# ErrorTzy/unpaper-gpu

Measured on AMD Instinct MI355X. Metric: pages/sec + Mpixel/s, 1000-page GRAY8 A4@300dpi batch, 1/2/4/8 GPU, higher is better.
Workload: dtype u8; 1 GPU; 1000 synthetic GRAY8 A4@300dpi pages (2480x3508) per GPU, default pipeline, inputs and outputs resident in HBM; pages_per_gpu=1000, sheets_per_batch=64, streams=16, hw_queues=24, parallelism=one runner thread per device, pages sharded, no collective

## Files before the change

unpaper-gpu_amd/csrc/kernels_noise.hip:

```cpp
#include "filters_common.h"

namespace uph {

constexpr int kNT = 64;
constexpr int kHalo = 14;
constexpr int kRW = kNT + 2 * kHalo;
constexpr int kNTG = 100;
template <int FMT>
constexpr int noise_tile_w() { return FMT == F_GRAY8 ? kNTG : kNT; }
constexpr int kZone = 32;
constexpr int kEligible = kZone + 8;

bool noise_geometry(int32_t W, int32_t H, uint64_t intensity, uint8_t white, NoiseGeom* g) {
  g->W = W;
  g->H = H;
  g->intensity = intensity > 64 ? 64 : (int32_t)intensity;
  g->white = white;
  g->all_seq = intensity > 4 ? 1 : 0;
  int64_t cap = g->all_seq ? (int64_t)W * H + 64 : ((int64_t)W * H) / 4 + 1024;
  if (cap > (1 << 27)) cap = 1 << 27;
  g->capacity = (int32_t)cap;
  return true;
}

static size_t noise_list_bytes(const NoiseGeom& g) {
  size_t b = 256 + (size_t)g.capacity * 4 * 2;
  return (b + 255) & ~(size_t)255;
}

static size_t pow2_at_least(size_t n) {
  size_t p = 1;
  while (p < n) p <<= 1;
  return p;
}

static int32_t noise_bit_words(const NoiseGeom& g) { return noise_bit_words(g.W); }

constexpr int kCapPerThread = 16;
static int group_threads(int32_t W, int32_t H) { return (int64_t)W * H > (16 << 20) ? 1024 : 256; }
size_t noise_scratch_bytes(const NoiseGeom& g) {
  size_t sort = 4 * pow2_at_least((size_t)g.capacity);
  const size_t cap3 = 12 * (size_t)kCapPerThread * (size_t)group_threads(g.W, g.H);
  if (sort < cap3) sort = cap3;
  const size_t bits = 4 * (size_t)noise_bit_words(g) * (size_t)g.H;
  return noise_list_bytes(g) + (sort > bits ? sort : bits);
}

struct NoisePtrs {
  uint32_t* nclear;
  uint32_t* nseq;
  uint32_t* clear;
  uint32_t* seq;
};
__device__ __forceinline__ NoisePtrs noise_ptrs(const NoiseGeom& g, uint8_t* base) {
  NoisePtrs p;
  p.nclear = (uint32_t*)base;
  p.nseq = p.nclear + 1;
  p.clear = (uint32_t*)(base + 256);
  p.seq = p.clear + g.capacity;
  return p;
}

__device__ __forceinline__ uint32_t row9(const uint32_t* w, int c) {
  const int word = c >> 5, off = c & 31;
  uint64_t v = ((uint64_t)w[word + 1] << 32) | w[word];
  return (uint32_t)(v >> off) & 0x1FFu;
}

__device__ __forceinline__ int flood9(const uint32_t (*drow)[4], int cx, int cy, uint32_t* comp) {
  uint32_t D[9], cur[9];
#pragma unroll
  for (int r = 0; r < 9; r++) {
    D[r] = row9(drow[cy - 4 + r], cx - 4);
    cur[r] = 0;
  }
  cur[4] = 1u << 4;
  for (int it = 0; it < 4; it++) {
    uint32_t nx[9];
    bool same = true;
    int n = 0;
#pragma unroll
    for (int r = 0; r < 9; r++) {
      uint32_t u = cur[r] | (r > 0 ? cur[r - 1] : 0) | (r < 8 ? cur[r + 1] : 0);
      u = (u | (u << 1) | (u >> 1)) & D[r] & 0x1FFu;
      nx[r] = u;
      same &= (u == cur[r]);
      n += __popc(u);
    }
#pragma unroll
    for (int r = 0; r < 9; r++) cur[r] = nx[r];
    if (n > 4) {
#pragma unroll
      for (int r = 0; r < 9; r++) comp[r] = cur[r];
      return n;
    }
    if (same) break;
  }
  int n = 0;
#pragma unroll
  for (int r = 0; r < 9; r++) {
    comp[r] = cur[r];
    n += __popc(cur[r]);
  }
  return n;
}

__device__ __forceinline__ uint32_t row_bits(const uint32_t* w, int c, int n) {
  const int word = c >> 5, off = c & 31;
  const uint64_t v = ((uint64_t)(word < 3 ? w[word + 1] : 0u) << 32) | w[word];
  return (uint32_t)(v >> off) & (n >= 32 ? 0xFFFFFFFFu : ((1u << n) - 1u));
}

__device__ __forceinline__ void wave_append(bool want, int32_t gx, int32_t gy, uint32_t* counter,
                                            uint32_t* list, int32_t capacity) {
  const unsigned long long M = __ballot(want);
  if (!M) return;
  const int lane = threadIdx.x & 63;
  uint32_t base = 0;
  const int leader = __ffsll((long long)M) - 1;
  if (lane == leader) base = atomicAdd(counter, (uint32_t)__popcll(M));
  base = __shfl(base, leader, 64);
  if (want) {
    const uint32_t k = base + (uint32_t)__popcll(M & ((1ull << lane) - 1ull));
    if (k < (uint32_t)capacity) list[k] = ((uint32_t)gy << 16) | (uint32_t)gx;
  }
}

__global__ void __launch_bounds__(256) k_noise_bits(PlaneRef img, NoiseGeom g, uint32_t* bits,
                                                    int64_t bstride, int32_t nwr, float rnwr) {
  const int s = blockIdx.y;
  const int32_t t = blockIdx.x * 256 + threadIdx.x;
  int32_t y = (int32_t)((float)t * rnwr);
  if (y * nwr > t) y--;
  else if ((y + 1) * nwr <= t) y++;
  if (y >= g.H) return;
  const int32_t wi = t - y * nwr, x0 = 32 * wi;
  const uint4* p = reinterpret_cast<const uint4*>(plane_ptr(img, s) + (int64_t)y * img.P.pitch + x0);
  const uint4 a = p[0], b = p[1];
  uint32_t m = dark_bits32({a.x, a.y, a.z, a.w, b.x, b.y, b.z, b.w}, g.white);
  if (x0 + 32 > g.W) m &= (1u << (g.W - x0)) - 1u;
  bits[s * bstride + t] = m;
}

struct SmallVerdict {
  bool seq, clear;
};
constexpr uint32_t kNotSmall = 0xFFFFFFFFu;
__device__ __forceinline__ uint32_t pack_comp(const uint32_t (&comp)[9]) {
  uint32_t rec = kNotSmall;
  int nc = 0;
#pragma unroll
  for (int r = 0; r < 9; r++) {
    uint32_t mm = comp[r];
    while (mm) {
      const int b = __ffs(mm) - 1;
      mm &= mm - 1;
      if (nc < 4) rec = (rec & ~(0xFFu << (8 * nc))) | ((uint32_t)(b | (r << 4)) << (8 * nc));
      nc++;
    }
  }
  return nc <= 4 ? rec : kNotSmall;
}
__device__ __forceinline__ SmallVerdict small_verdict_pixels(const uint32_t (*drow)[4],
                                                             const uint32_t (*trow)[4],
                                                             const uint32_t (*srow)[4], int rx,
                                                             int ry, int32_t gx, int32_t gy,
                                                             bool trig, int N, int nc,
                                                             const int (&cxs)[4],
                                                             const int (&cys)[4]) {
  SmallVerdict v{false, false};
  int bx0 = 4, bx1 = -4, by0 = 4, by1 = -4;
#pragma unroll
  for (int k = 0; k < 4; k++)
    if (k < nc) {
      bx0 = imin(bx0, cxs[k]);
      bx1 = imax(bx1, cxs[k]);
      by0 = imin(by0, cys[k]);
      by1 = imax(by1, cys[k]);
    }
  bool eligible = nc <= 4 && gx + bx0 >= kEligible && gy + by0 >= kEligible;
  if (eligible) {
    const int X0 = rx + bx0 - 7, n = bx1 - bx0 + 15;
    const int r0 = ry + by0 - 7, r1 = ry + by1 + 7;
    int cnt = 0;
#pragma unroll
    for (int j = 0; j < 18; j++)
      if (r0 + j <= r1) cnt += __popc(row_bits(srow[r0 + j], X0, n));
    eligible = cnt == nc;
  }
  if (!eligible) {
    v.seq = trig;
    return v;
  }
  for (int k = 0; k < nc && k < 4 && !v.clear; k++) {
    const int cx = rx + (k == 0 ? cxs[0] : k == 1 ? cxs[1] : k == 2 ? cxs[2] : cxs[3]);
    const int cy = ry + (k == 0 ? cys[0] : k == 1 ? cys[1] : k == 2 ? cys[2] : cys[3]);
    if (!((trow[cy][cx >> 5] >> (cx & 31)) & 1)) continue;
    uint32_t D[9];
#pragma unroll
    for (int r = 0; r < 9; r++) D[r] = row_bits(drow[cy - 4 + r], cx - 4, 9);
    int count = 1;
    bool go = true;
#pragma unroll
    for (int L = 1; L <= 4; L++) {
      if (!go || L > N) break;
      const uint32_t span = ((1u << (2 * L + 1)) - 1u) << (4 - L);
      const uint32_t ends = (1u << (4 - L)) | (1u << (4 + L));
      int lc = __popc(D[4 - L] & span) + __popc(D[4 + L] & span);
#pragma unroll
      for (int r = 4 - L + 1; r <= 4 + L - 1; r++) lc += __popc(D[r] & ends);
      count += lc;
      go = lc != 0;
    }
    v.clear = count <= N;
  }
  return v;
}
__device__ __forceinline__ SmallVerdict small_verdict_rec(const uint32_t (*drow)[4],
                                                          const uint32_t (*trow)[4],
                                                          const uint32_t (*srow)[4], int rx, int ry,
                                                          int32_t gx, int32_t gy, bool trig, int N,
                                                          uint32_t rec) {
  int cxs[4], cys[4], nc = 0;
#pragma unroll
  for (int k = 0; k < 4; k++) {
    const uint32_t b = (rec >> (8 * k)) & 0xFFu;
    cxs[k] = (int)(b & 15u) - 4;
    cys[k] = (int)(b >> 4) - 4;
    nc += b != 0xFFu;
  }
  return small_verdict_pixels(drow, trow, srow, rx, ry, gx, gy, trig, N, nc, cxs, cys);
}
__device__ __forceinline__ SmallVerdict small_verdict(const uint32_t (*drow)[4],
                                                      const uint32_t (*trow)[4],
                                                      const uint32_t (*srow)[4], int rx, int ry,
                                                      int32_t gx, int32_t gy, bool trig, int N) {
  uint32_t comp[9];
  flood9(drow, rx, ry, comp);
  const uint32_t rec = pack_comp(comp);
  if (rec == kNotSmall) return SmallVerdict{trig, false};
  return small_verdict_rec(drow, trow, srow, rx, ry, gx, gy, trig, N, rec);
}

constexpr int kListCap = 1024;

#ifndef UPH_CLASSIFY_OCC
#define UPH_CLASSIFY_OCC 8
#endif
template <int FMT>
__global__ void __launch_bounds__(256, UPH_CLASSIFY_OCC) k_noise_classify(PlaneRef img, NoiseGeom g, uint8_t* scratch,
                                                        int64_t sstride, SheetCtl* ctl,
                                                        const uint32_t* bits, int64_t bstride) {
  int bxi, byi, s;
  xcd_block(&bxi, &byi, &s);
  constexpr int NTX = noise_tile_w<FMT>();
  constexpr int RWX = NTX + 2 * kHalo;
  static_assert(RWX > 64 && RWX <= 128, "region rows are two 64-bit halves");
  const int32_t tx0 = bxi * NTX, ty0 = byi * kNT;
  const int32_t ox = tx0 - kHalo, oy = ty0 - kHalo;
  const uint8_t* base = plane_ptr(img, s);
  NoisePtrs NP = noise_ptrs(g, scratch + s * sstride);
  const int lane = threadIdx.x & 63, w = threadIdx.x >> 6;
  constexpr bool kGray = FMT == F_GRAY8;
  constexpr bool kSplit = FMT == F_RGB24;
  constexpr uint64_t kIn0 = ~0ull << kHalo;
  constexpr uint64_t kIn1 = (1ull << (kHalo + NTX - 64)) - 1ull;
  __shared__ uint32_t drow[kRW][4];
  __shared__ uint32_t trow_s[kSplit ? kRW : 1][4];
  __shared__ uint32_t srow[kRW][4];
  __shared__ uint64_t l3[kRW][2], cand[kRW][2];
  __shared__ uint16_t wl[kListCap];
  __shared__ uint32_t crec[kListCap];
  __shared__ int32_t any_dark, nwl;
  uint32_t (*trow)[4] = kSplit ? trow_s : drow;
  constexpr int B = FMT == F_GRAY8 ? 1 : FMT == F_Y400A ? 2 : 3;
  const int64_t pitch = img.P.pitch;
  if (threadIdx.x == 0) {
    any_dark = 0;
    nwl = 0;
  }
  for (int i = threadIdx.x; i < kRW * 4; i += 256) (&srow[0][0])[i] = 0;
  if constexpr (kGray) {
    bool dark_here = false;
    if (threadIdx.x < kRW) {
      const int ry = threadIdx.x;
      const int32_t gy = oy + ry;
      const int32_t nwr = (g.W + 31) >> 5;
      const int32_t wb = ox >> 5;
      const int sh = ox & 31;
      uint32_t q[5] = {0u, 0u, 0u, 0u, 0u};
      if (gy >= 0 && gy < g.H) {
        const uint32_t* row = bits + s * bstride + (int64_t)gy * nwr;
#pragma unroll
        for (int j = 0; j < 5; j++)
          if (wb + j >= 0 && wb + j < nwr) q[j] = row[wb + j];
      }
      uint32_t d[4];
#pragma unroll
      for (int j = 0; j < 4; j++) d[j] = __builtin_amdgcn_alignbit(q[j + 1], q[j], sh);
      if (RWX < 128) {
        if (RWX <= 96) {
          d[2] &= RWX > 64 ? (1u << (RWX - 64)) - 1u : 0u;
          d[3] = 0u;
        } else {
          d[3] &= (1u << (RWX - 96)) - 1u;
        }
      }
#pragma unroll
      for (int j = 0; j < 4; j++) drow[ry][j] = d[j];
      const uint64_t lo64 = ((uint64_t)d[1] << 32) | d[0], hi64 = ((uint64_t)d[3] << 32) | d[2];
      dark_here = ry >= kHalo && ry < kHalo + kNT && ((lo64 & kIn0) | (hi64 & kIn1));
    }
    __syncthreads();
    if (dark_here) any_dark = 1;
  } else {
    constexpr int NV = (RWX * B + 30) / 16;
    constexpr int NLOAD = (kRW * NV + 255) / 256;
    __shared__ uint4 stage[kRW][NV];
    const int64_t sb = (int64_t)ox * B;
    const int64_t a0 = sb >= 0 ? (sb & ~(int64_t)15) : -((-sb + 15) & ~(int64_t)15);
    uint4 v[NLOAD];
#pragma unroll
    for (int k = 0; k < NLOAD; k++) {
      const int i = threadIdx.x + k * 256;
      const int ry = i / NV, vi = i % NV;
      const int32_t gy = oy + ry;
      const int64_t off = a0 + 16 * vi;
      v[k] = make_uint4(0, 0, 0, 0);
      if (i < kRW * NV && gy >= 0 && gy < g.H && off >= 0 && off < pitch)
        v[k] = *reinterpret_cast<const uint4*>(base + (int64_t)gy * pitch + off);
    }
#pragma unroll
    for (int k = 0; k < NLOAD; k++) {
      const int i = threadIdx.x + k * 256;
      if (i < kRW * NV) stage[i / NV][i % NV] = v[k];
    }
    __syncthreads();
    const int lead = (int)(sb - a0);
    bool colok[2];
    int rxc[2];
#pragma unroll
    for (int h = 0; h < 2; h++) {
      const int rx = h * 64 + lane;
      colok[h] = (rx < RWX) & (ox + rx >= 0) & (ox + rx < g.W);
      rxc[h] = rx < RWX ? rx : 0;
    }
    bool tile_dark = false;
    for (int ry = w; ry < kRW; ry += 4) {
      const int32_t gy = oy + ry;
      const bool rowok = (gy >= 0) & (gy < g.H);
      const uint8_t* srow_b = reinterpret_cast<const uint8_t*>(stage[ry]) + lead;
      unsigned long long md[2], mt[2];
#pragma unroll
      for (int h = 0; h < 2; h++) {
        const bool in = colok[h] & rowok;
        if constexpr (kSplit) {
          const Px p = load_px_row<FMT>(srow_b, rxc[h]);
          md[h] = __ballot(in & (light_of(p) < g.white));
          mt[h] = __ballot(in & (dark_of(p) < g.white));
        } else {
          const uint32_t v = srow_b[rxc[h] * B];
          md[h] = mt[h] = __ballot(in & (v < (uint32_t)g.white));
        }
      }
      if (lane < 4) {
        const unsigned long long q = md[lane >> 1];
        drow[ry][lane] = (uint32_t)(lane & 1 ? q >> 32 : q);
        if (kSplit) {
          const unsigned long long t = mt[lane >> 1];
          trow[ry][lane] = (uint32_t)(lane & 1 ? t >> 32 : t);
        }
      }
      if (ry >= kHalo && ry < kHalo + kNT && ((md[0] & kIn0) | (md[1] & kIn1))) tile_dark = true;
    }
    if (lane == 0 && tile_dark) any_dark = 1;
  }
  __syncthreads();
  if (!any_dark) return;
  if (UPH_DIAG_BITS(g.diag, 3) == 1) return;
  const int hr = threadIdx.x >> 1, hh = threadIdx.x & 1;
  auto dark64 = [&](int r, int h) -> uint64_t {
    return ((uint64_t)drow[r][2 * h + 1] << 32) | drow[r][2 * h];
  };
  if (threadIdx.x < 2 * kRW) {
    uint64_t c0 = 0, c1 = 0, c2 = 0, c3 = 0;
#pragma unroll
    for (int d = -1; d <= 1; d++) {
      const int r = hr + d;
      uint64_t v0 = 0, v1 = 0;
      if (r >= 0 && r < kRW) {
        v0 = dark64(r, 0);
        v1 = dark64(r, 1);
      }
      const uint64_t v = hh ? v1 : v0;
      const uint64_t Lw = hh ? (v1 << 1) | (v0 >> 63) : v0 << 1;
      const uint64_t Rw = hh ? v1 >> 1 : (v0 >> 1) | (v1 << 63);
      const uint64_t s0 = v ^ Lw ^ Rw;
      const uint64_t s1 = (v & Lw) | (v & Rw) | (Lw & Rw);
      const uint64_t k0 = c0 & s0;
      c0 ^= s0;
      const uint64_t t1 = c1 ^ s1;
      const uint64_t k1 = (c1 & s1) | (t1 & k0);
      c1 = t1 ^ k0;
      const uint64_t k2 = c2 & k1;
      c2 ^= k1;
      c3 |= k2;
    }
    l3[hr][hh] = dark64(hr, hh) & (c3 | (c2 & (c1 | c0)));
  }
  __syncthreads();
  if (threadIdx.x < 2 * kRW) {
    uint64_t c = 0;
    if (hr >= 4 && hr < kRW - 4) {
      uint64_t dil = 0;
#pragma unroll
      for (int d = -1; d <= 1; d++) {
        const uint64_t a0 = l3[hr + d][0], a1 = l3[hr + d][1];
        dil |= hh ? a1 | (a1 << 1) | (a0 >> 63) | (a1 >> 1) : a0 | (a0 << 1) | (a0 >> 1) | (a1 << 63);
      }
      c = dark64(hr, hh) & ~dil & (hh ? (1ull << (RWX - 4 - 64)) - 1ull : ~0xFull);
    }
    cand[hr][hh] = c;
    if (c) {
      int k = atomicAdd(&nwl, __popcll(c));
      while (c) {
        const int b = __ffsll((long long)c) - 1;
        c &= c - 1;
        if (k < kListCap) wl[k] = (uint16_t)((hr << 8) | (hh * 64 + b));
        k++;
      }
    }
  }
  __syncthreads();
  if (UPH_DIAG_BITS(g.diag, 3) == 2) return;
  const int ncand = nwl;
  if (ncand <= kListCap) {
    for (int i = threadIdx.x; i < ncand; i += 256) {
      const int e = wl[i], ry = e >> 8, rx = e & 0xFF;
      uint32_t comp[9];
      const bool small = flood9(drow, rx, ry, comp) <= 4;
      crec[i] = small ? pack_comp(comp) : kNotSmall;
      if (small) atomicOr(&srow[ry][rx >> 5], 1u << (rx & 31));
    }
  } else {
    for (int ry = w; ry < kRW; ry += 4) {
      unsigned long long m[2] = {0, 0};
#pragma unroll
      for (int h = 0; h < 2; h++) {
        const uint64_t c = cand[ry][h];
        if (!c) continue;
        bool small = false;
        if ((c >> lane) & 1) {
          uint32_t comp[9];
          small = flood9(drow, h * 64 + lane, ry, comp) <= 4;
        }
        m[h] = __ballot(small);
      }
      if (lane < 4) {
        const unsigned long long q = m[lane >> 1];
        srow[ry][lane] = (uint32_t)(lane & 1 ? q >> 32 : q);
      }
    }
  }
  __syncthreads();
  if (UPH_DIAG_BITS(g.diag, 3) == 3) return;
  const int N = g.intensity;
  const bool zone_tile = g.all_seq || tx0 < kZone || ty0 < kZone;
  if (zone_tile) {
    for (int t = w; t < kNT; t += 4) {
#pragma unroll 1
      for (int h = 0; h < (NTX + 63) / 64; h++) {
        const int ry = kHalo + t, cx = h * 64 + lane, rx = kHalo + (cx < NTX ? cx : 0);
        const int32_t gy = oy + ry, gx = ox + rx;
        const bool trig = (trow[ry][rx >> 5] >> (rx & 31)) & 1;
        const bool zone = g.all_seq || gx < kZone || gy < kZone;
        const bool dark = (drow[ry][rx >> 5] >> (rx & 31)) & 1;
        const bool noop = !g.all_seq && gx >= 8 && gy >= 7 && ((l3[ry][rx >> 6] >> (rx & 63)) & 1);
        wave_append(cx < NTX && dark & zone & trig & !noop, gx, gy, NP.nseq, NP.seq, g.capacity);
      }
    }
  }
  if (ncand <= kListCap) {
    for (int b0 = 0; b0 < ncand; b0 += 256) {
      const int i = b0 + threadIdx.x;
      SmallVerdict v{false, false};
      int32_t gx = 0, gy = 0;
      if (i < ncand) {
        const uint32_t rec = crec[i];
        const int e = wl[i], ry = e >> 8, rx = e & 0xFF;
        gx = ox + rx;
        gy = oy + ry;
        const bool inside = ry >= kHalo && ry < kHalo + kNT && rx >= kHalo && rx < kHalo + NTX;
        if (rec != kNotSmall && inside && !g.all_seq && gx >= kZone && gy >= kZone) {
          const bool trig = (trow[ry][rx >> 5] >> (rx & 31)) & 1;
          v = small_verdict_rec(drow, trow, srow, rx, ry, gx, gy, trig, N, rec);
        }
      }
      wave_append(v.seq, gx, gy, NP.nseq, NP.seq, g.capacity);
      wave_append(v.clear, gx, gy, NP.nclear, NP.clear, g.capacity);
    }
    return;
  }
  if (threadIdx.x == 0) nwl = 0;
  __syncthreads();
  constexpr int kChunks = (NTX + 31) / 32;
  static_assert(kChunks * kNT <= 256, "one thread per chunk");
  if (threadIdx.x < kChunks * kNT) {
    const int ry = kHalo + (threadIdx.x / kChunks), h = threadIdx.x % kChunks;
    uint32_t m = row_bits(srow[ry], kHalo + 32 * h, imin(32, NTX - 32 * h));
    if (m && !g.all_seq && oy + ry >= kZone) {
      const int32_t gx0 = ox + kHalo + 32 * h;
      if (gx0 < kZone) m &= kZone - gx0 >= 32 ? 0u : ~((1u << (kZone - gx0)) - 1u);
      if (m) {
        int k = atomicAdd(&nwl, __popc(m));
        while (m) {
          const int b = __ffs(m) - 1;
          m &= m - 1;
          if (k < kListCap) wl[k] = (uint16_t)((ry << 8) | (kHalo + 32 * h + b));
          k++;
        }
      }
    }
  }
  __syncthreads();
  const int nsmall = nwl;
  if (nsmall <= kListCap) {
    for (int b0 = 0; b0 < nsmall; b0 += 256) {
      const int i = b0 + threadIdx.x;
      SmallVerdict v{false, false};
      int32_t gx = 0, gy = 0;
      if (i < nsmall) {
        const int e = wl[i], ry = e >> 8, rx = e & 0xFF;
        gx = ox + rx;
        gy = oy + ry;
        const bool trig = (trow[ry][rx >> 5] >> (rx & 31)) & 1;
        v = small_verdict(drow, trow, srow, rx, ry, gx, gy, trig, N);
      }
      wave_append(v.seq, gx, gy, NP.nseq, NP.seq, g.capacity);
      wave_append(v.clear, gx, gy, NP.nclear, NP.clear, g.capacity);
    }
  } else {
    for (int t = w; t < kNT; t += 4) {
      const int ry = kHalo + t;
      uint32_t any = 0;
#pragma unroll
      for (int h = 0; h < kChunks; h++) any |= row_bits(srow[ry], kHalo + 32 * h, imin(32, NTX - 32 * h));
      if (!any) continue;
#pragma unroll 1
      for (int h = 0; h < (NTX + 63) / 64; h++) {
        const int cx = h * 64 + lane, rx = kHalo + (cx < NTX ? cx : 0);
        const int32_t gy = oy + ry, gx = ox + rx;
        const bool zone = g.all_seq || gx < kZone || gy < kZone;
        const bool small = cx < NTX && !zone && ((srow[ry][rx >> 5] >> (rx & 31)) & 1);
        SmallVerdict v{false, false};
        if (small) {
          const bool trig = (trow[ry][rx >> 5] >> (rx & 31)) & 1;
          v = small_verdict(drow, trow, srow, rx, ry, gx, gy, trig, N);
        }
        wave_append(v.seq, gx, gy, NP.nseq, NP.seq, g.capacity);
        wave_append(v.clear, gx, gy, NP.nclear, NP.clear, g.capacity);
      }
    }
  }
}

template <int FMT>
__device__ __forceinline__ uint32_t* sheet_bb(const NoiseGeom& g, int s) {
  return FMT == F_GRAY8 && g.bbits ? g.bbits + s * g.bb_stride : nullptr;
}
__device__ __forceinline__ void bb_clear(uint32_t* bb, int32_t W, int32_t x, int32_t y) {
  if (bb) atomicAnd(bb + (int64_t)y * ((W + 31) >> 5) + (x >> 5), ~(1u << (x & 31)));
}

template <int FMT>
__global__ void __launch_bounds__(256) k_noise_apply(PlaneRef img, NoiseGeom g, uint8_t* scratch,
                                                     int64_t sstride, SheetCtl* ctl) {
  const int s = blockIdx.y;
  NoisePtrs NP = noise_ptrs(g, scratch + s * sstride);
  const uint32_t n = *NP.nclear;
  if (n > (uint32_t)g.capacity) {
    if (blockIdx.x == 0 && threadIdx.x == 0 && ctl) atomicOr(&ctl[s].status, STATUS_NOISE_OVERFLOW);
    return;
  }
  uint8_t* base = plane_ptr(img, s);
  uint32_t* bb = sheet_bb<FMT>(g, s);
  for (uint32_t i = blockIdx.x * 256 + threadIdx.x; i < n; i += gridDim.x * 256) {
    const uint32_t k = NP.clear[i];
    white_px<FMT>(base + (int64_t)(k >> 16) * img.P.pitch, (int32_t)(k & 0xFFFF));
    bb_clear(bb, g.W, (int32_t)(k & 0xFFFF), (int32_t)(k >> 16));
  }
}

__device__ void block_sort(uint32_t* a, int n_pow2) {
  for (int k = 2; k <= n_pow2; k <<= 1) {
    int j = k >> 1;
    for (; j >= 64; j >>= 1) {
      for (int i = threadIdx.x; i < n_pow2; i += blockDim.x) {
        const int l = i ^ j;
        if (l > i) {
          const uint32_t x = a[i], y = a[l];
          const bool up = (i & k) == 0;
          if ((x > y) == up) {
            a[i] = y;
            a[l] = x;
          }
        }
      }
      __threadfence_block();
      __syncthreads();
    }
    for (int i = threadIdx.x; i < n_pow2; i += blockDim.x) {
      uint32_t x = a[i];
      const bool up = (i & k) == 0;
      for (int jj = j; jj > 0; jj >>= 1) {
        const uint32_t y = (uint32_t)__shfl_xor((int)x, jj, 64);
        const bool lower = (i & jj) == 0;
        x = lower == up ? (x < y ? x : y) : (x < y ? y : x);
      }
      a[i] = x;
    }
    __threadfence_block();
    __syncthreads();
  }
}

__device__ __forceinline__ bool ring_pos(int L, int k, int* dx, int* dy) {
  const int row = 2 * L + 1, col = 2 * L - 1;
  if (k < row) {
    *dx = k - L;
    *dy = -L;
  } else if (k < 2 * row) {
    *dx = k - row - L;
    *dy = L;
  } else if (k < 2 * row + col) {
    *dx = -L;
    *dy = k - 2 * row - (L - 1);
  } else if (k < 2 * row + 2 * col) {
    *dx = L;
    *dy = k - 2 * row - col - (L - 1);
  } else {
    return false;
  }
  return true;
}

__device__ __forceinline__ bool ring_member(int L, int dx, int dy, int32_t x, int32_t y) {
  return iabs(dy) == L ? x >= L : y >= L - 1;
}

struct Mask81 {
  uint64_t lo;
  uint32_t hi;
};
__device__ __forceinline__ Mask81 ring_part(int L, bool rows) {
  Mask81 m{0, 0};
#pragma unroll
  for (int p = 0; p < 81; p++) {
    const int dx = p % 9 - 4, dy = p / 9 - 4;
    const int adx = iabs(dx), ady = iabs(dy);
    const bool on = rows ? (ady == L && adx <= L) : (adx == L && ady < L);
    if (on) {
      if (p < 64) m.lo |= 1ull << p;
      else m.hi |= 1u << (p - 64);
    }
  }
  return m;
}

template <int FMT>
__device__ __forceinline__ void replay_trigger4(int32_t x, int32_t y, int N, const NoiseGeom& g,
                                                uint8_t* base, int64_t pitch,
                                                const Mask81 (&rowp)[5], const Mask81 (&colp)[5],
                                                uint32_t* bb) {
  uint64_t dlo = 0;
  uint32_t dhi = 0;
  bool ctr = false;
  if constexpr (FMT == F_GRAY8) {
    const int32_t c0 = x - 4;
    const int32_t d0 = c0 >= 0 ? (c0 & ~3) : -(((-c0) + 3) & ~3);
    const int32_t dmax = (int32_t)pitch - 4;
    uint32_t w[9][3];
#pragma unroll
    for (int r = 0; r < 9; r++) {
      const uint8_t* row = base + (int64_t)imin(imax(y + r - 4, 0), g.H - 1) * pitch;
#pragma unroll
      for (int j = 0; j < 3; j++)
        w[r][j] = *reinterpret_cast<const uint32_t*>(row + imin(imax(d0 + 4 * j, 0), dmax));
    }
    const int o = c0 - d0;
#pragma unroll
    for (int p = 0; p < 81; p++) {
      const int r = p / 9, c = p % 9;
      const int32_t qx = c0 + c, qy = y + r - 4;
      const bool in = (qx >= 0) & (qy >= 0) & (qx < g.W) & (qy < g.H);
      const int b = o + c;
      const uint32_t wd = b < 4 ? w[r][0] : b < 8 ? w[r][1] : w[r][2];
      const uint32_t v = (wd >> (8 * (b & 3))) & 0xFFu;
      const bool dk = in & (v < g.white);
      if (p < 64) dlo |= (uint64_t)dk << p;
      else dhi |= (uint32_t)dk << (p - 64);
      if (p == 40) ctr = v < g.white;
    }
  } else if constexpr (FMT == F_RGB24) {
    const int32_t b0 = 3 * (x - 4);
    const int32_t d0 = b0 >= 0 ? (b0 & ~3) : -(((-b0) + 3) & ~3);
    const int32_t dmax = (int32_t)pitch - 4;
    const int o = b0 - d0;
#pragma unroll
    for (int r = 0; r < 9; r++) {
      const uint8_t* row = base + (int64_t)imin(imax(y + r - 4, 0), g.H - 1) * pitch;
      uint32_t w[8], a[7];
#pragma unroll
      for (int j = 0; j < 8; j++)
        w[j] = *reinterpret_cast<const uint32_t*>(row + imin(imax(d0 + 4 * j, 0), dmax));
#pragma unroll
// ... 322 lines not shown
    const int kb = nl <= kLongList ? (int)longs[q++] : k++;
    const int lo = (int)bc[kb], len = (int)bc[kb + 1] - lo;
    if (len <= kGroupBucketMax) continue;
    int p2 = 1;
    while (p2 < len) p2 <<= 1;
    __threadfence_block();
    __syncthreads();
    if (!BIG || p2 <= kCompCap) {
      for (int i = tid; i < p2; i += kGroupThreads) cur[i] = i < len ? keys[lo + i] : 0xFFFFFFFFu;
      __threadfence_block();
      __syncthreads();
      block_sort(cur, p2);
      for (int i = tid; i < len; i += kGroupThreads) keys[lo + i] = cur[i];
    } else {
      uint32_t* stage = NP.clear;
      for (int i = tid; i < p2; i += kGroupThreads) stage[i] = i < len ? keys[lo + i] : 0xFFFFFFFFu;
      __threadfence_block();
      __syncthreads();
      block_sort(stage, p2);
      for (int i = tid; i < len; i += kGroupThreads) keys[lo + i] = stage[i];
    }
  }
  __threadfence_block();
  __syncthreads();
  uint32_t* par = big ? NP.seq : cur;
  for (int i = tid; i < (int)n; i += kGroupThreads) par[i] = (uint32_t)i;
  __threadfence_block();
  __syncthreads();
  for (int i = tid; i < (int)n; i += kGroupThreads) {
    const uint32_t key = keys[i];
    const int32_t x = (int32_t)(key & 0xFFFF), y = (int32_t)(key >> 16);
    for (int j = (int)bc[imax(y - R, 0) >> b]; j < i; j++) {
      const uint32_t kj = keys[j];
      const int32_t xj = (int32_t)(kj & 0xFFFF), yj = (int32_t)(kj >> 16);
      if (yj >= y - R && xj >= x - R && xj <= x + R) {
        if (big) uf_union<true>(par, (uint32_t)i, (uint32_t)j);
        else uf_union(par, (uint32_t)i, (uint32_t)j);
      }
    }
  }
  __threadfence_block();
  __syncthreads();
  if (!big) {
    for (int i = tid; i < (int)n; i += kGroupThreads) {
      gk[i] = keys[i];
      gk[kCompCap + i] = uf_find(par, (uint32_t)i);
    }
    __syncthreads();
    for (int i = tid; i < (int)n; i += kGroupThreads) keys[i] = 0u;
    __syncthreads();
    for (int i = tid; i < (int)n; i += kGroupThreads) atomicMax(&keys[gk[kCompCap + i]], (uint32_t)i);
    __syncthreads();
    for (int i = tid; i < (int)n; i += kGroupThreads) gk[2 * kCompCap + i] = keys[i];
    if (tid == 0) *flag = kNoiseLds;
    return;
  }
  uint32_t* last = NP.clear;
  for (int i = tid; i < (int)n; i += kGroupThreads) last[i] = 0u;
  for (int i = tid; i < (int)n; i += kGroupThreads) par[i] = uf_find<true>(par, (uint32_t)i);
  __threadfence_block();
  __syncthreads();
  for (int i = tid; i < (int)n; i += kGroupThreads) atomicMax(&last[par[i]], (uint32_t)i);
  __threadfence();
  __syncthreads();
  if (tid == 0) *flag = kNoiseBig;
}

template <int FMT, int T>
__global__ void __launch_bounds__(T) k_noise_group(PlaneRef img, NoiseGeom g, uint8_t* scratch,
                                                   int64_t sstride, SheetCtl* ctl,
                                                   uint32_t* sortbuf, int64_t sort_stride) {
  constexpr int kCompCap = kCapPerThread * T;
  const int s = blockIdx.x;
  NoisePtrs NP = noise_ptrs(g, scratch + s * sstride);
  uint32_t* flag = NP.nclear + 2;
  const uint32_t n = *NP.nseq;
  const int N = g.intensity;
  const int tid = threadIdx.x;
#ifdef UPHIP_DIAG
  if ((g.diag & 8) && tid == 0) printf("uphip noise: sheet %d seq %u clear %u\n", s, n, *NP.nclear);
#endif
  if (n == 0 || n > (uint32_t)g.capacity) {
    if (tid == 0) {
      *flag = kNoiseNothing;
      if (n != 0 && ctl) atomicOr(&ctl[s].status, STATUS_NOISE_OVERFLOW);
    }
    return;
  }
  uint32_t* gk = sortbuf + s * sort_stride;
  extern __shared__ uint32_t glds[];
  uint8_t* base = plane_ptr(img, s);
  const int64_t pitch = img.P.pitch;
  uint32_t* bb = sheet_bb<FMT>(g, s);
  if (N > 4) {
    int p2 = 1;
    while (p2 < (int)n) p2 <<= 1;
    if (tid == 0) *flag = kNoiseNothing;
    if (p2 <= kCompCap) noise_raster_replay<FMT>(glds, (int)n, p2, g, NP, base, pitch, bb);
    else noise_raster_replay<FMT>(gk, (int)n, p2, g, NP, base, pitch, bb);
    return;
  }
  if (n > (uint32_t)kCompCap)
    noise_group_sheet<FMT, T, true>(g, NP, gk, glds, base, pitch, flag, n, bb);
  else
    noise_group_sheet<FMT, T, false>(g, NP, gk, glds, base, pitch, flag, n, bb);
}

template <int FMT>
__global__ void __launch_bounds__(256) k_noise_replay(PlaneRef img, NoiseGeom g, uint8_t* scratch,
                                                      int64_t sstride, const uint32_t* sortbuf,
                                                      int64_t sort_stride, int kCompCap) {
  const int s = blockIdx.y;
  NoisePtrs NP = noise_ptrs(g, scratch + s * sstride);
  const uint32_t n = *NP.nseq;
  const uint32_t layout = NP.nclear[2];
  if (layout == kNoiseNothing || blockIdx.x * blockDim.x >= n) return;
  const uint32_t* keys = sortbuf + s * sort_stride;
  const uint32_t* root = layout == kNoiseLds ? keys + kCompCap : NP.seq;
  const uint32_t* last = layout == kNoiseLds ? keys + 2 * kCompCap : NP.clear;
  Mask81 rowp[5], colp[5];
#pragma unroll
  for (int L = 1; L <= 4; L++) {
    rowp[L] = ring_part(L, true);
    colp[L] = ring_part(L, false);
  }
  uint8_t* base = plane_ptr(img, s);
  uint32_t* bb = sheet_bb<FMT>(g, s);
  for (int i = blockIdx.x * blockDim.x + threadIdx.x; i < (int)n; i += gridDim.x * blockDim.x) {
    if (root[i] != (uint32_t)i) continue;
    const int end = (int)last[i];
    for (int j = i; j <= end; j++) {
      if (root[j] != (uint32_t)i) continue;
      const uint32_t key = keys[j];
      __threadfence_block();
      replay_trigger4<FMT>((int32_t)(key & 0xFFFF), (int32_t)(key >> 16), g.intensity, g, base,
                           img.P.pitch, rowp, colp, bb);
    }
  }
}

__global__ void k_noise_zero(uint8_t* scr, int64_t stride, int count) {
  const int s = blockIdx.x * blockDim.x + threadIdx.x;
  if (s < count) {
    uint32_t* c = (uint32_t*)(scr + s * stride);
    c[0] = 0;
    c[1] = 0;
  }
}

template <int FMT>
static void launch_noise_t(const PlaneRef& img, const NoiseGeom& g, uint8_t* scr, int64_t ss,
                           SheetCtl* ctl, int count, hipStream_t st, uint32_t* sortbuf,
                           int64_t sort_stride, const SheetBits& ready) {
  constexpr int ntx = noise_tile_w<FMT>();
  dim3 grid((g.W + ntx - 1) / ntx, (g.H + kNT - 1) / kNT, count);
  NoiseGeom gd = g;
  gd.diag = diag_noise();
  gd.bbits = ready.bbits;
  gd.bb_stride = ready.stride;
  uint32_t* bits = ready.nbits;
  int64_t bstride = ready.stride;
  if (FMT == F_GRAY8 && !bits) {
    const int32_t nwr = noise_bit_words(g);
    bits = sortbuf;
    bstride = sort_stride;
    const int64_t words = (int64_t)nwr * g.H;
    hipLaunchKernelGGL(k_noise_bits, dim3((unsigned)((words + 255) / 256), count), dim3(256), 0, st,
                       img, g, bits, bstride, nwr, 1.0f / (float)nwr);
  }
  UPH_LAUNCH_DIAG(131072, k_noise_classify<FMT>, grid, dim3(256), 0, st, img, gd, scr, ss, ctl,
                     bits, bstride);
  hipLaunchKernelGGL(k_noise_apply<FMT>, dim3(64, count), dim3(256), 0, st, img, gd, scr, ss, ctl);
  const int gt = group_threads(g.W, g.H);
  if (!(diag_skip() & 2)) {
    if (gt == 1024) {
      allow_dynamic_lds((const void*)k_noise_group<FMT, 1024>, group_lds(1024));
      hipLaunchKernelGGL((k_noise_group<FMT, 1024>), dim3(count), dim3(1024), group_lds(1024), st, img, gd,
                         scr, ss, ctl, sortbuf, sort_stride);
    } else {
      allow_dynamic_lds((const void*)k_noise_group<FMT, 256>, group_lds(256));
      hipLaunchKernelGGL((k_noise_group<FMT, 256>), dim3(count), dim3(256), group_lds(256), st, img, gd,
                         scr, ss, ctl, sortbuf, sort_stride);
    }
    hipLaunchKernelGGL(k_noise_replay<FMT>, dim3(replay_blocks(count), count), dim3(256), 0, st, img,
                       gd, scr, ss, sortbuf, sort_stride, kCapPerThread * gt);
  }
}

void launch_noisefilter(const PlaneRef& img, const NoiseGeom& g, void* scratch,
                        int64_t scratch_stride, SheetCtl* ctl, int count, hipStream_t st,
                        const SheetBits& bits) {
  uint8_t* scr = (uint8_t*)scratch;
  const size_t lists = noise_list_bytes(g);
  uint32_t* sortbuf = (uint32_t*)(scr + lists);
  const int64_t sort_stride = scratch_stride / 4;
  hipLaunchKernelGGL(k_noise_zero, dim3((count + 255) / 256), dim3(256), 0, st, scr,
                     scratch_stride, count);
  switch (img.P.fmt) {
    case F_GRAY8:
      launch_noise_t<F_GRAY8>(img, g, scr, scratch_stride, ctl, count, st, sortbuf, sort_stride,
                              bits);
      break;
    case F_Y400A:
      launch_noise_t<F_Y400A>(img, g, scr, scratch_stride, ctl, count, st, sortbuf, sort_stride,
                              {});
      break;
    default:
      launch_noise_t<F_RGB24>(img, g, scr, scratch_stride, ctl, count, st, sortbuf, sort_stride,
                              {});
      break;
  }
}

}
```

Baseline: 29330 pages/s.

## Classify GRAY8 noise on global bit-plane with candidate and verdict kernels

For GRAY8 the tiled classify kernel with halo regions is replaced by two plane-wide kernels. The first computes candidates and zone-sequential pixels with bit-sliced row arithmetic per 32-bit word strip and writes a small-component bit-plane. The second runs the verdict only on the set small bits and appends to both output lists through a single combined ballot. This removes the halo recomputation and the shared-memory staging per tile, at the cost of an extra intermediate plane in scratch (scratch size doubled) and one more kernel launch. Other formats keep the old tiled path.

```diff
diff --git a/unpaper-gpu_amd/csrc/kernels_noise.hip b/unpaper-gpu_amd/csrc/kernels_noise.hip
--- a/unpaper-gpu_amd/csrc/kernels_noise.hip
+++ b/unpaper-gpu_amd/csrc/kernels_noise.hip
@@ -1,15 +1,13 @@
 #include "filters_common.h"
+#include "noise_planes.h"
 
 namespace uph {
 
 constexpr int kNT = 64;
 constexpr int kHalo = 14;
 constexpr int kRW = kNT + 2 * kHalo;
-constexpr int kNTG = 100;
-template <int FMT>
-constexpr int noise_tile_w() { return FMT == F_GRAY8 ? kNTG : kNT; }
-constexpr int kZone = 32;
-constexpr int kEligible = kZone + 8;
+constexpr int kZone = kNpZone;
+constexpr int kEligible = kNpEligible;
 
 bool noise_geometry(int32_t W, int32_t H, uint64_t intensity, uint8_t white, NoiseGeom* g) {
   g->W = W;
@@ -42,7 +40,7 @@
   size_t sort = 4 * pow2_at_least((size_t)g.capacity);
   const size_t cap3 = 12 * (size_t)kCapPerThread * (size_t)group_threads(g.W, g.H);
   if (sort < cap3) sort = cap3;
-  const size_t bits = 4 * (size_t)noise_bit_words(g) * (size_t)g.H;
+  const size_t bits = 2 * 4 * (size_t)noise_bit_words(g) * (size_t)g.H;
   return noise_list_bytes(g) + (sort > bits ? sort : bits);
 }
 
@@ -124,6 +122,26 @@
     const uint32_t k = base + (uint32_t)__popcll(M & ((1ull << lane) - 1ull));
     if (k < (uint32_t)capacity) list[k] = ((uint32_t)gy << 16) | (uint32_t)gx;
   }
+}
+
+__device__ __forceinline__ void wave_append2(bool want1, bool want2, int32_t gx, int32_t gy,
+                                             uint32_t* counter1, uint32_t* list1,
+                                             uint32_t* counter2, uint32_t* list2,
+                                             int32_t capacity) {
+  const unsigned long long M1 = __ballot(want1), M2 = __ballot(want2);
+  if (!(M1 | M2)) return;
+  const int lane = threadIdx.x & 63;
+  uint32_t b1 = 0, b2 = 0;
+  if (lane == 0) {
+    if (M1) b1 = atomicAdd(counter1, (uint32_t)__popcll(M1));
+    if (M2) b2 = atomicAdd(counter2, (uint32_t)__popcll(M2));
+  }
+  b1 = __shfl(b1, 0, 64);
+  b2 = __shfl(b2, 0, 64);
+  const unsigned long long below = (1ull << lane) - 1ull;
+  const uint32_t k = want1 ? b1 + (uint32_t)__popcll(M1 & below) : b2 + (uint32_t)__popcll(M2 & below);
+  if ((want1 | want2) && k < (uint32_t)capacity)
+    (want1 ? list1 : list2)[k] = ((uint32_t)gy << 16) | (uint32_t)gx;
 }
 
 __global__ void __launch_bounds__(256) k_noise_bits(PlaneRef img, NoiseGeom g, uint32_t* bits,
@@ -249,11 +267,11 @@
 #endif
 template <int FMT>
 __global__ void __launch_bounds__(256, UPH_CLASSIFY_OCC) k_noise_classify(PlaneRef img, NoiseGeom g, uint8_t* scratch,
-                                                        int64_t sstride, SheetCtl* ctl,
-                                                        const uint32_t* bits, int64_t bstride) {
+                                                        int64_t sstride, SheetCtl* ctl) {
+  static_assert(FMT != F_GRAY8, "GRAY8 classifies its bit-plane: k_noise_cand, k_noise_verdict");
   int bxi, byi, s;
   xcd_block(&bxi, &byi, &s);
-  constexpr int NTX = noise_tile_w<FMT>();
+  constexpr int NTX = kNT;
   constexpr int RWX = NTX + 2 * kHalo;
   static_assert(RWX > 64 && RWX <= 128, "region rows are two 64-bit halves");
   const int32_t tx0 = bxi * NTX, ty0 = byi * kNT;
@@ -261,7 +279,6 @@
   const uint8_t* base = plane_ptr(img, s);
   NoisePtrs NP = noise_ptrs(g, scratch + s * sstride);
   const int lane = threadIdx.x & 63, w = threadIdx.x >> 6;
-  constexpr bool kGray = FMT == F_GRAY8;
   constexpr bool kSplit = FMT == F_RGB24;
   constexpr uint64_t kIn0 = ~0ull << kHalo;
   constexpr uint64_t kIn1 = (1ull << (kHalo + NTX - 64)) - 1ull;
@@ -273,47 +290,14 @@
   __shared__ uint32_t crec[kListCap];
   __shared__ int32_t any_dark, nwl;
   uint32_t (*trow)[4] = kSplit ? trow_s : drow;
-  constexpr int B = FMT == F_GRAY8 ? 1 : FMT == F_Y400A ? 2 : 3;
+  constexpr int B = FMT == F_Y400A ? 2 : 3;
   const int64_t pitch = img.P.pitch;
   if (threadIdx.x == 0) {
     any_dark = 0;
     nwl = 0;
   }
   for (int i = threadIdx.x; i < kRW * 4; i += 256) (&srow[0][0])[i] = 0;
-  if constexpr (kGray) {
-    bool dark_here = false;
-    if (threadIdx.x < kRW) {
-      const int ry = threadIdx.x;
-      const int32_t gy = oy + ry;
-      const int32_t nwr = (g.W + 31) >> 5;
-      const int32_t wb = ox >> 5;
-      const int sh = ox & 31;
-      uint32_t q[5] = {0u, 0u, 0u, 0u, 0u};
-      if (gy >= 0 && gy < g.H) {
-        const uint32_t* row = bits + s * bstride + (int64_t)gy * nwr;
-#pragma unroll
-        for (int j = 0; j < 5; j++)
-          if (wb + j >= 0 && wb + j < nwr) q[j] = row[wb + j];
-      }
-      uint32_t d[4];
-#pragma unroll
-      for (int j = 0; j < 4; j++) d[j] = __builtin_amdgcn_alignbit(q[j + 1], q[j], sh);
-      if (RWX < 128) {
-        if (RWX <= 96) {
-          d[2] &= RWX > 64 ? (1u << (RWX - 64)) - 1u : 0u;
-          d[3] = 0u;
-        } else {
-          d[3] &= (1u << (RWX - 96)) - 1u;
-        }
-      }
-#pragma unroll
-      for (int j = 0; j < 4; j++) drow[ry][j] = d[j];
-      const uint64_t lo64 = ((uint64_t)d[1] << 32) | d[0], hi64 = ((uint64_t)d[3] << 32) | d[2];
-      dark_here = ry >= kHalo && ry < kHalo + kNT && ((lo64 & kIn0) | (hi64 & kIn1));
-    }
-    __syncthreads();
-    if (dark_here) any_dark = 1;
-  } else {
+  {
     constexpr int NV = (RWX * B + 30) / 16;
     constexpr int NLOAD = (kRW * NV + 255) / 256;
     __shared__ uint4 stage[kRW][NV];
@@ -561,6 +545,144 @@
         wave_append(v.clear, gx, gy, NP.nclear, NP.clear, g.capacity);
       }
     }
+  }
+}
+
+constexpr int kPRA = 16;
+constexpr int kPRB = 16;
+constexpr int kPList = 1024;
+constexpr uint32_t kPZone = 1u << 18;
+
+struct PlaneThread {
+  int32_t wi, y0;
+};
+template <int R>
+__device__ __forceinline__ PlaneThread plane_thread(int32_t t, int32_t nwr, float rnwr) {
+  int32_t q = (int32_t)((float)t * rnwr);
+  if (q * nwr > t) q--;
+  else if ((q + 1) * nwr <= t) q++;
+  return PlaneThread{t - q * nwr, q * R};
+}
+
+__device__ __forceinline__ uint32_t list_append(uint32_t m, int r, uint32_t kind, int32_t* nwl,
+                                                uint32_t* wl) {
+  if (!m) return 0u;
+  int k = atomicAdd(nwl, __popc(m));
+  while (m && k < kPList) {
+    const int b = __ffs(m) - 1;
+    m &= m - 1;
+    wl[k++] = (uint32_t)b | (threadIdx.x << 5) | ((uint32_t)r << 13) | kind;
+  }
+  return m;
+}
+
+__global__ void __launch_bounds__(256) k_noise_cand(NoiseGeom g, uint8_t* scratch, int64_t sstride,
+                                                    const uint32_t* bits, int64_t bstride,
+                                                    uint32_t* small, int64_t small_stride,
+                                                    int32_t nwr, float rnwr) {
+  const int s = blockIdx.y;
+  const NpPlane P{bits + s * bstride, nwr, g.H};
+  NoisePtrs NP = noise_ptrs(g, scratch + s * sstride);
+  const int32_t t0 = blockIdx.x * 256;
+  const PlaneThread me = plane_thread<kPRA>(t0 + threadIdx.x, nwr, rnwr);
+  __shared__ uint32_t smallw[kPRA][256];
+  __shared__ uint32_t wl[kPList];
+  __shared__ int32_t nwl;
+  uint32_t cand[kPRA], zone[kPRA];
+  {
+    uint32_t l3[kPRA];
+    if (me.y0 < g.H) {
+      np_strip<kPRA>(P, me.wi, me.y0, g.all_seq, l3, cand, zone);
+    } else {
+#pragma unroll
+      for (int r = 0; r < kPRA; r++) cand[r] = zone[r] = 0u;
+    }
+  }
+#pragma unroll
+  for (int r = 0; r < kPRA; r++) {
+    smallw[r][threadIdx.x] = 0u;
+    if (g.all_seq) cand[r] = 0u;
+  }
+  for (;;) {
+    if (threadIdx.x == 0) nwl = 0;
+    __syncthreads();
+#pragma unroll
+    for (int r = 0; r < kPRA; r++) {
+      cand[r] = list_append(cand[r], r, 0u, &nwl, wl);
+      zone[r] = list_append(zone[r], r, kPZone, &nwl, wl);
+    }
+    __syncthreads();
+    const int tot = nwl, n = imin(tot, kPList);
+    for (int b0 = 0; b0 < n; b0 += 256) {
+      const int i = b0 + threadIdx.x;
+      bool seq = false;
+      int32_t gx = 0, gy = 0;
+      if (i < n) {
+        const uint32_t e = wl[i];
+        const int et = (e >> 5) & 255, r = (e >> 13) & 31;
+        const PlaneThread o = plane_thread<kPRA>(t0 + et, nwr, rnwr);
+        gx = 32 * o.wi + (int32_t)(e & 31u);
+        gy = o.y0 + r;
+        seq = e & kPZone;
+        if (!seq) {
+          uint32_t comp[9], D[9];
+          if (np_flood9(P, gx, gy, comp, D) <= kNpSmallMax) atomicOr(&smallw[r][et], 1u << (e & 31u));
+        }
+      }
+      wave_append(seq, gx, gy, NP.nseq, NP.seq, g.capacity);
+    }
+    __syncthreads();
+    if (tot <= kPList) break;
+  }
+  if (g.all_seq || me.y0 >= g.H) return;
+  uint32_t* out = small + s * small_stride + (int64_t)me.y0 * nwr + me.wi;
+#pragma unroll
+  for (int r = 0; r < kPRA; r++)
+    if (me.y0 + r < g.H) out[(int64_t)r * nwr] = smallw[r][threadIdx.x];
+}
+
+__global__ void __launch_bounds__(256) k_noise_verdict(NoiseGeom g, uint8_t* scratch,
+                                                       int64_t sstride, const uint32_t* bits,
+                                                       int64_t bstride, const uint32_t* small,
+                                                       int64_t small_stride, int32_t nwr,
+                                                       float rnwr) {
+  const int s = blockIdx.y;
+  const NpPlane P{bits + s * bstride, nwr, g.H};
+  const NpPlane S{small + s * small_stride, nwr, g.H};
+  NoisePtrs NP = noise_ptrs(g, scratch + s * sstride);
+  const int32_t t0 = blockIdx.x * 256;
+  const PlaneThread me = plane_thread<kPRB>(t0 + threadIdx.x, nwr, rnwr);
+  __shared__ uint32_t wl[kPList];
+  __shared__ int32_t nwl;
+  uint32_t todo[kPRB];
+#pragma unroll
+  for (int r = 0; r < kPRB; r++) {
+    const int32_t y = me.y0 + r;
+    todo[r] = me.wi > 0 && y >= kNpZone && y < g.H ? S.w[(int64_t)y * nwr + me.wi] : 0u;
+  }
+  for (;;) {
+    if (threadIdx.x == 0) nwl = 0;
+    __syncthreads();
+#pragma unroll
+    for (int r = 0; r < kPRB; r++) todo[r] = list_append(todo[r], r, 0u, &nwl, wl);
+    __syncthreads();
+    const int tot = nwl, n = imin(tot, kPList);
+    for (int b0 = 0; b0 < n; b0 += 256) {
+      const int i = b0 + threadIdx.x;
+      int v = NP_NONE;
+      int32_t gx = 0, gy = 0;
+      if (i < n) {
+        const uint32_t e = wl[i];
+        const PlaneThread o = plane_thread<kPRB>(t0 + (int)((e >> 5) & 255), nwr, rnwr);
+        gx = 32 * o.wi + (int32_t)(e & 31u);
+        gy = o.y0 + (int)((e >> 13) & 31);
+        v = np_verdict(P, S, gx, gy, g.intensity);
+      }
+      wave_append2(v == NP_SEQ, v == NP_CLEAR, gx, gy, NP.nseq, NP.seq, NP.nclear, NP.clear,
+                   g.capacity);
+    }
+    __syncthreads();
+    if (tot <= kPList) break;
   }
 }
 
@@ -1189,24 +1311,35 @@
 static void launch_noise_t(const PlaneRef& img, const NoiseGeom& g, uint8_t* scr, int64_t ss,
                            SheetCtl* ctl, int count, hipStream_t st, uint32_t* sortbuf,
                            int64_t sort_stride, const SheetBits& ready) {
-  constexpr int ntx = noise_tile_w<FMT>();
-  dim3 grid((g.W + ntx - 1) / ntx, (g.H + kNT - 1) / kNT, count);
   NoiseGeom gd = g;
   gd.diag = diag_noise();
   gd.bbits = ready.bbits;
   gd.bb_stride = ready.stride;
-  uint32_t* bits = ready.nbits;
-  int64_t bstride = ready.stride;
-  if (FMT == F_GRAY8 && !bits) {
+  if constexpr (FMT == F_GRAY8) {
     const int32_t nwr = noise_bit_words(g);
-    bits = sortbuf;
-    bstride = sort_stride;
     const int64_t words = (int64_t)nwr * g.H;
-    hipLaunchKernelGGL(k_noise_bits, dim3((unsigned)((words + 255) / 256), count), dim3(256), 0, st,
-                       img, g, bits, bstride, nwr, 1.0f / (float)nwr);
-  }
-  UPH_LAUNCH_DIAG(131072, k_noise_classify<FMT>, grid, dim3(256), 0, st, img, gd, scr, ss, ctl,
-                     bits, bstride);
+    const uint32_t* bits = ready.nbits;
+    int64_t bstride = ready.stride;
+    uint32_t* small = sortbuf;
+    if (!bits) {
+      hipLaunchKernelGGL(k_noise_bits, dim3((unsigned)((words + 255) / 256), count), dim3(256), 0, st,
+                         img, g, sortbuf, sort_stride, nwr, 1.0f / (float)nwr);
+      bits = sortbuf;
+      bstride = sort_stride;
+      small = sortbuf + words;
+    }
+    const int64_t ta = (int64_t)nwr * ((g.H + kPRA - 1) / kPRA);
+    const int64_t tb = (int64_t)nwr * ((g.H + kPRB - 1) / kPRB);
+    const dim3 grid((unsigned)((ta + 255) / 256), count), gridb((unsigned)((tb + 255) / 256), count);
+    UPH_LAUNCH_DIAG(131072, k_noise_cand, grid, dim3(256), 0, st, gd, scr, ss, bits, bstride, small,
+                    sort_stride, nwr, 1.0f / (float)nwr);
+    if (!g.all_seq)
+      UPH_LAUNCH_DIAG(131072, k_noise_verdict, gridb, dim3(256), 0, st, gd, scr, ss, bits, bstride,
+                      small, sort_stride, nwr, 1.0f / (float)nwr);
+  } else {
+    dim3 grid((g.W + kNT - 1) / kNT, (g.H + kNT - 1) / kNT, count);
+    UPH_LAUNCH_DIAG(131072, k_noise_classify<FMT>, grid, dim3(256), 0, st, img, gd, scr, ss, ctl);
+  }
   hipLaunchKernelGGL(k_noise_apply<FMT>, dim3(64, count), dim3(256), 0, st, img, gd, scr, ss, ctl);
   const int gt = group_threads(g.W, g.H);
   if (!(diag_skip() & 2)) {
diff --git a/unpaper-gpu_amd/csrc/noise_planes.h b/unpaper-gpu_amd/csrc/noise_planes.h
--- /dev/null
+++ b/unpaper-gpu_amd/csrc/noise_planes.h
@@ -0,0 +1,231 @@
+#ifndef UNPAPER_HIP_NOISE_PLANES_H
+#define UNPAPER_HIP_NOISE_PLANES_H
+
+#include <stdint.h>
+
+#ifdef __HIPCC__
+#define NP_FN __host__ __device__ static inline
+#else
+#define NP_FN static inline
+#endif
+
+enum {
+  kNpZone = 32,
+  kNpEligible = 40,
+  kNpSmallMax = 4
+};
+
+typedef struct NpPlane {
+  const uint32_t* w;
+  int32_t nwr, H;
+} NpPlane;
+
+NP_FN int np_popc(uint32_t v) {
+#ifdef __HIP_DEVICE_COMPILE__
+  return __popc(v);
+#else
+  return __builtin_popcount(v);
+#endif
+}
+NP_FN int np_ctz(uint32_t v) {
+#ifdef __HIP_DEVICE_COMPILE__
+  return __ffs((int)v) - 1;
+#else
+  return __builtin_ctz(v);
+#endif
+}
+
+NP_FN uint32_t np_word(const NpPlane P, int32_t wi, int32_t y) {
+  const int32_t cw = wi < 0 ? 0 : wi >= P.nwr ? P.nwr - 1 : wi;
+  const int32_t cy = y < 0 ? 0 : y >= P.H ? P.H - 1 : y;
+  const uint32_t v = P.w[(int64_t)cy * P.nwr + cw];
+  return ((cw == wi) & (cy == y)) ? v : 0u;
+}
+
+NP_FN uint32_t np_bits(const NpPlane P, int32_t x, int32_t y, int n) {
+  const int32_t wi = x >> 5;
+  const int off = x & 31;
+  const uint64_t v = np_word(P, wi, y) | ((uint64_t)np_word(P, wi + 1, y) << 32);
+  return (uint32_t)(v >> off) & (n >= 32 ? 0xFFFFFFFFu : ((1u << n) - 1u));
+}
+
+typedef struct NpRow {
+  uint32_t v, s0, s1;
+  uint32_t hl, hr;
+  uint32_t dl, dr;
+} NpRow;
+NP_FN NpRow np_row(const NpPlane P, int32_t wi, int32_t y) {
+  const uint32_t l = np_word(P, wi - 1, y), v = np_word(P, wi, y), r = np_word(P, wi + 1, y);
+  const uint32_t L = (v << 1) | (l >> 31), R = (v >> 1) | (r << 31);
+  NpRow o;
+  o.v = v;
+  o.s0 = v ^ L ^ R;
+  o.s1 = (v & L) | (v & R) | (L & R);
+  o.hl = (uint32_t)np_popc((l >> 30) | ((v & 1u) << 2));
+  o.hr = (uint32_t)np_popc((v >> 31) | ((r & 3u) << 1));
+  o.dl = l >> 31;
+  o.dr = r & 1u;
+  return o;
+}
+
+NP_FN uint32_t np_l3(const NpRow a, const NpRow b, const NpRow c, uint32_t* edge) {
+  const uint32_t t0 = a.s0 ^ b.s0 ^ c.s0;
+  const uint32_t k0 = (a.s0 & b.s0) | (a.s0 & c.s0) | (b.s0 & c.s0);
+  const uint32_t x = a.s1 ^ b.s1 ^ c.s1;
+  const uint32_t m = (a.s1 & b.s1) | (a.s1 & c.s1) | (b.s1 & c.s1);
+  const uint32_t u1 = x ^ k0, k1 = x & k0;
+  const uint32_t u2 = m ^ k1, u3 = m & k1;
+  *edge = (b.dl & (uint32_t)(a.hl + b.hl + c.hl >= 5u)) |
+          ((b.dr & (uint32_t)(a.hr + b.hr + c.hr >= 5u)) << 1);
+  return b.v & (u3 | (u2 & (u1 | t0)));
+}
+
+NP_FN uint32_t np_cand(uint32_t v, uint32_t la, uint32_t lb, uint32_t lc, uint32_t ea,
+                       uint32_t eb, uint32_t ec) {
+  const uint32_t o = la | lb | lc, e = ea | eb | ec;
+  return v & ~(o | (o << 1) | (o >> 1) | (e & 1u) | ((e >> 1) << 31));
+}
+
+NP_FN uint32_t np_zone(uint32_t dark, uint32_t l3, int32_t wi, int32_t y, int all_seq) {
+  if (all_seq) return dark;
+  const uint32_t in = y < kNpZone || wi == 0 ? 0xFFFFFFFFu : 0u;
+  const uint32_t noop = y >= 7 ? (wi == 0 ? 0xFFFFFF00u : 0xFFFFFFFFu) : 0u;
+  return dark & in & ~(l3 & noop);
+}
+
+template <int R>
+NP_FN void np_strip(const NpPlane P, int32_t wi, int32_t y0, int all_seq, uint32_t* l3w,
+                    uint32_t* candw, uint32_t* zonew) {
+  NpRow ra = np_row(P, wi, y0 - 2), rb = np_row(P, wi, y0 - 1), rc = np_row(P, wi, y0);
+  uint32_t ea, eb, ec;
+  uint32_t la = np_l3(ra, rb, rc, &ea);
+  ra = rb;
+  rb = rc;
+  rc = np_row(P, wi, y0 + 1);
+  uint32_t lb = np_l3(ra, rb, rc, &eb);
+#if defined(__clang__)
+#pragma unroll
+#endif
+  for (int r = 0; r < R; r++) {
+    ra = rb;
+    rb = rc;
+    rc = np_row(P, wi, y0 + r + 2);
+    const uint32_t lc = np_l3(ra, rb, rc, &ec);
+    l3w[r] = lb;
+    candw[r] = np_cand(ra.v, la, lb, lc, ea, eb, ec);
+    zonew[r] = np_zone(ra.v, lb, wi, y0 + r, all_seq);
+    la = lb;
+    lb = lc;
+    ea = eb;
+    eb = ec;
+  }
+}
+
+NP_FN int np_flood9(const NpPlane P, int32_t x, int32_t y, uint32_t* comp, uint32_t* D) {
+  uint32_t cur[9];
+#if defined(__clang__)
+#pragma unroll
+#endif
+  for (int r = 0; r < 9; r++) {
+    D[r] = np_bits(P, x - 4, y - 4 + r, 9);
+    cur[r] = 0;
+  }
+  cur[4] = 1u << 4;
+  int n = 1;
+  for (int it = 0; it < 4; it++) {
+    uint32_t nx[9];
+    int same = 1;
+    n = 0;
+#if defined(__clang__)
+#pragma unroll
+#endif
+    for (int r = 0; r < 9; r++) {
+      uint32_t u = cur[r] | (r > 0 ? cur[r - 1] : 0) | (r < 8 ? cur[r + 1] : 0);
+      u = (u | (u << 1) | (u >> 1)) & D[r];
+      nx[r] = u;
+      same &= (u == cur[r]);
+      n += np_popc(u);
+    }
+#if defined(__clang__)
+#pragma unroll
+#endif
+    for (int r = 0; r < 9; r++) cur[r] = nx[r];
+    if (n > kNpSmallMax || same) break;
+  }
+#if defined(__clang__)
+#pragma unroll
+#endif
+  for (int r = 0; r < 9; r++) comp[r] = cur[r];
+  return n;
+}
+
+NP_FN int np_ring_test(const uint32_t* D, int N) {
+  int count = 1, go = 1;
+#if defined(__clang__)
+#pragma unroll
+#endif
+  for (int L = 1; L <= 4; L++) {
+    if (!go || L > N) break;
+    const uint32_t span = ((1u << (2 * L + 1)) - 1u) << (4 - L);
+    const uint32_t ends = (1u << (4 - L)) | (1u << (4 + L));
+    int lc = np_popc(D[4 - L] & span) + np_popc(D[4 + L] & span);
+    for (int r = 4 - L + 1; r <= 4 + L - 1; r++) lc += np_popc(D[r] & ends);
+    count += lc;
+    go = lc != 0;
+  }
+  return count <= N;
+}
+
+enum { NP_NONE = 0, NP_SEQ = 1, NP_CLEAR = 2 };
+
+NP_FN int np_verdict(const NpPlane dark, const NpPlane small, int32_t x, int32_t y, int N) {
+  uint32_t comp[9], D[9];
+  if (np_flood9(dark, x, y, comp, D) > kNpSmallMax) return NP_SEQ;
+  int by0 = 4, by1 = -4, nc = 0;
+  uint32_t any = 0;
+#if defined(__clang__)
+#pragma unroll
+#endif
+  for (int r = 0; r < 9; r++) {
+    if (comp[r]) {
+      if (by0 > r - 4) by0 = r - 4;
+      by1 = r - 4;
+      any |= comp[r];
+      nc += np_popc(comp[r]);
+    }
+  }
+  const int bx0 = np_ctz(any) - 4, bx1 = 27 - (int)__builtin_clz(any);
+  if (x + bx0 < kNpEligible || y + by0 < kNpEligible) return NP_SEQ;
+  {
+    const int32_t X0 = x + bx0 - 7;
+    const int n = bx1 - bx0 + 15;
+    const int32_t r0 = y + by0 - 7, r1 = y + by1 + 7;
+    int cnt = 0;
+#if defined(__clang__)
+#pragma unroll
+#endif
+    for (int j = 0; j < 18; j++) {
+      const int c = np_popc(np_bits(small, X0, r0 + j, n));
+      cnt += r0 + j <= r1 ? c : 0;
+    }
+    if (cnt != nc) return NP_SEQ;
+  }
+  if (np_ring_test(D, N)) return NP_CLEAR;
+  comp[4] &= ~(1u << 4);
+  for (int cr = 1; cr < 8; cr++) {
+    uint32_t m = comp[cr];
+    while (m) {
+      const int cb = np_ctz(m);
+      m &= m - 1;
+      const int32_t cx = x + cb - 4, cy = y + cr - 4;
+#if defined(__clang__)
+#pragma unroll
+#endif
+      for (int r = 0; r < 9; r++) D[r] = np_bits(dark, cx - 4, cy - 4 + r, 9);
+      if (np_ring_test(D, N)) return NP_CLEAR;
+    }
+  }
+  return NP_NONE;
+}
+
+#endif
```

Result: faster. 31800 pages/s, median of 6 (+8.4%).
